# 21K1113/Neural_Image_Compression_V2

Measured on AMD Instinct MI355X. Metric: Mpixels/sec train-step (fwd+bwd) + PSNR, 4K RGB, 1/2/4/8 MI355X, higher is better.
Workload: dtype bf16x2-split operands, f32 accumulate

## Files before the change

### ab/w16/scratch_depth.py

```python
import re, sys, collections
kern, depth = None, 0
acc, mfma = collections.defaultdict(list), collections.defaultdict(collections.Counter)
for l in open(sys.argv[1]):
    m = re.match(r"^(_ZN3nic\w+):", l)
    if m:
        kern, depth = (re.sub(r".*LayoutILi(\d)EEELi(\d).*", r"Layout<\1>, MODE \2", m.group(1)) if "fused_train16" in m.group(1) else None), 0
        continue
    if kern is None:
        continue
    if re.match(r"^(\.LBB\d+_\d+:|; %bb\.\d+:)", l):
        d = re.search(r"Depth=(\d+)", l)
        depth = int(d.group(1)) if d else 0
    elif "scratch_" in l:
        acc[kern].append((depth, l.split()[0]))
    elif "v_mfma" in l:
        mfma[kern][depth] += 1
for k in mfma:
    print(f"{k}: MFMAs by depth {dict(mfma[k])}; scratch accesses by depth {dict(collections.Counter(d for d, _ in acc[k]))}"
          f"{'  <-- IN THE ROUND LOOP' if any(d >= 3 for d, _ in acc[k]) else ''}")
```

### ab/w16/stamps16.py

```python
import os, sys, ctypes
sys.path.insert(0, os.path.dirname(os.path.dirname(os.path.dirname(os.path.abspath(__file__)))))
import torch, numpy as np
from neural_image_compression_v2_amd import _lib, fused, fp_def
from neural_image_compression_v2_amd.image_compression import ColorDecoder
dev = torch.device("cuda:0")
torch.manual_seed(0)
H, W = 2160, 3840
NS = H * W
fp, _ = fp_def.create_pyramid((H // 4, W // 4), 12, 8, dev, torch.float32, True)
dec = ColorDecoder(73, 64).to(dev)
geo = fused.PathGeometry(dim=2, method=1, step_number=0.25, mip_level=0, extent=(H, W), num_crops=1,
                         noise_mode=int(os.environ.get("NOISE", "2")), noise_seed=7, noise_offset=1,
                         flags=_lib.NIC_FLAG_ORIGINS_ALIGNED, split_bf16=True)
org = torch.zeros(1, 2, dtype=torch.int32, device=dev)
params = [p.detach() for p in dec.linear_params()]
target = torch.rand(NS, 3, device=dev)
for _ in range(3):
    out = fused.fused_forward_backward(geo, fp[0].detach(), fp[1].detach(), org, params, target)
torch.cuda.synchronize()
d = geo.to_desc(fp[0], fp[1])
ws = _lib.workspace(dev, int(_lib.load().nic_workspace_bytes(ctypes.byref(d))))
REC, NWG = 20992, 256
off = NWG * REC * 4
st = ws[off:off + NWG * 8 * 16 * 8].view(torch.int64).view(NWG * 8, 16).cpu().numpy().astype(np.float64)
names = ["0 coords, blend, PE, noise", "1 L1, L2, L3 (+ image stores, GELUs)", "2 dZ3 image, dW3, dA2", "3 dA1 (+ dZ2 image), db2", "4 wait barrier 1",
         "5 dW2 MFMAs", "6 wait barrier 2", "7 dX (+ dZ1 image), grid acc", "8 wait barrier 3", "9 dW1 MFMAs", "10 wait barrier 4", "11 -",
         "12 macro-tile setup", "13 grid flush"]
tot = st[:, :14].sum(1)
print(f"waves {st.shape[0]}, total cycles/wave median {np.median(tot):.3e} (min {tot.min():.3e}, max {tot.max():.3e})")
rounds = NS / 16 / (NWG * 8)
for i, n in enumerate(names):
    print(f"{n:40s} {100 * np.median(st[:, i] / tot):6.2f} %   {np.median(st[:, i]) / rounds:9.0f} cycles/round")
wave_id = np.arange(st.shape[0]) % 8
for kh in (0, 1):
    sel = (wave_id >> 2) == kh
    print(f"-- half {kh}: total cycles/wave median {np.median(tot[sel]):.3e}")
    for i, n in enumerate(names):
        print(f"   {n:40s} {np.median(st[sel, i]) / rounds:9.0f} cycles/round")
```

### neural_image_compression_v2_amd/csrc/fused_train16.hpp

```cpp
#pragma once
#include "fused_kernel.hpp"


#ifndef NIC_T16_HALF16
#define NIC_T16_HALF16 1
#endif
#ifndef NIC_T16_LOFF
#define NIC_T16_LOFF 26
#endif
#ifndef NIC_T16_PIN
#define NIC_T16_PIN 0
#endif
namespace nic {

struct Lds16 {
    static constexpr int LD1 = 80, LD2 = 80, LD3 = 80;
    static constexpr int LDZ = 72, LDX = 88;
    static constexpr int KP = 80;
    static constexpr int OFF_W1 = 0;
    static constexpr int W1LO = kH * LD1;
    static constexpr int OFF_W2 = OFF_W1 + 2 * kH * LD1;
    static constexpr int W2LO = kH * LD2;
    static constexpr int OFF_W3 = OFF_W2 + 2 * kH * LD2;
    static constexpr int W3LO = 4 * LD3;
// ... 52 lines not shown
__device__ __forceinline__ Frag2 split_pair(const f32x4& a, const f32x4& b) {
    const float x[8] = {a[0], a[1], a[2], a[3], b[0], b[1], b[2], b[3]};
    return split8(x);
}
__device__ __forceinline__ lds_bf* opaque(lds_bf* p) {
#ifndef NIC_NO_OPAQUE_PTR
    asm volatile("" : "+v"(p));
#endif
    return p;
}

#ifndef NIC_T16_PF
#define NIC_T16_PF 2
#endif
template <int NT, bool ZERO = false, class LoadA>
__device__ __forceinline__ void kstep16(f32x4 (&acc)[NT], const Frag2& bf, LoadA&& load_a) {
    constexpr int PF = NIC_T16_PF < NT ? NIC_T16_PF : NT;
    Frag2 af[PF];
#pragma unroll
    for (int t = 0; t < PF; ++t) af[t] = load_a(t);
#pragma unroll
    for (int t = 0; t < NT; ++t) {
        acc[t] = mfma16_split(af[t % PF], bf, ZERO ? f32x4(0.f) : acc[t]);
        if (t + PF < NT) af[t % PF] = load_a(t + PF);
    }
}

struct CellRaw16 {
    float g0[kC];
    float g1[4 * 3];
};
struct GridAcc16 {
    float g1[4 * 3];
};

__device__ __forceinline__ int opaque_i(int v) {
#ifndef NIC_NO_OPAQUE_LANE
    asm volatile("" : "+v"(v));
#endif
    return v;
}

__device__ __forceinline__ float grid_load16(const char* base, uint32_t ob, int kind, const FusedParams& p) {
    if (kind == 0) return *reinterpret_cast<const float*>(base + ob);
    if (kind == 3) {
        const float n = (float)*reinterpret_cast<const uint8_t*>(base + ob) - p.dq_sub;
        const float q = mul_rn(n, p.dq_rcp);
        return fmaf(fmaf(-q, p.dq_den, n), p.dq_rcp, q);
    }
    const uint32_t hbits = *reinterpret_cast<const uint16_t*>(base + ob);
    if (kind == 1) return __builtin_bit_cast(float, hbits << 16);
    return (float)__builtin_bit_cast(_Float16, (uint16_t)hbits);
}
__device__ __forceinline__ void gather_cell16(const FusedParams& p, uint32_t off0, uint32_t off1, int g, CellRaw16& raw) {
    const int kind = p.grid_kind;
    const uint32_t eb = kind == 0 ? 4u : (kind == 3 ? 1u : 2u);
    const uint32_t pb0 = (uint32_t)p.g0.plane * eb, pb1 = (uint32_t)p.g1.plane * eb;
    {
        uint32_t ob = (off0 + (uint32_t)p.g0.at(g >> 1, g & 1, 0)) * eb;
        const char* base = reinterpret_cast<const char*>(p.g0.p);
#pragma unroll
        for (int c = 0; c < kC; ++c, ob += pb0) raw.g0[c] = grid_load16(base, ob, kind, p);
    }
#pragma unroll
    for (int c4 = 0; c4 < 4; ++c4) {
        uint32_t ob = (off1 + (uint32_t)p.g1.at(c4 >> 1, c4 & 1, 0)) * eb + (uint32_t)(3 * g) * pb1;
        const char* base = reinterpret_cast<const char*>(p.g1.p);
#pragma unroll
        for (int cc = 0; cc < 3; ++cc, ob += pb1) raw.g1[c4 * 3 + cc] = grid_load16(base, ob, kind, p);
    }
}

template <class L>
__device__ __forceinline__ void encode16(const FusedParams& p, const int (&q)[3], int g, float (&xs)[20], EncCtx& cx, const CellRaw16& raw) {
    const nic_path_desc& d = p.d;
    const int e = d.log2_step;
    const Axis ax = axis_coords(q[0], e), ay = axis_coords(q[1], e);
    cx.kx = ax.k1; cx.ky = ay.k1; cx.kz = 0.f;
#pragma unroll
    for (int c = 0; c < kC; ++c) xs[c] = raw.g0[c];
    {
        const float c = (g >> 1) ? ay.t1 : ax.t1;
#pragma unroll
        for (int i = 0; i < 3; ++i) {
            const int r = 3 * (g & 1) + i;
            float v;
            if (L::PE == NIC_PE_TRIANGULAR) {
                v = tri_pe_row(c, r, kP);
            } else {
                const int k = r >> 1;
                const float dv = k == 0 ? d.pe_div[0] : (k == 1 ? d.pe_div[1] : d.pe_div[2]);
                float sv, cv;
                sincos_cw(mul_rn(c, dv), sv, cv);
                v = (r & 1) ? cv : sv;
            }
            xs[15 + i] = v;
        }
        xs[18] = g == 0 ? d.lod_value : (g == 1 ? 1.0f : 0.f);
    }
    const G1FactorsT<2> gf = g1_factors<2>(d.g1_weight_mode, cx.kx, cx.ky, 0.f);
#pragma unroll
    for (int cc = 0; cc < 3; ++cc) {
        float sum = 0.f;
#pragma unroll
        for (int c4 = 0; c4 < 4; ++c4) {
            const uint32_t b = (gf.bits >> (3 * c4)) & 7u;
            float v = raw.g1[c4 * 3 + cc];
            v = mul_rn(v, (b & 1u) ? gf.fx[1] : gf.fx[0]);
            v = mul_rn(v, (b & 2u) ? gf.fy[1] : gf.fy[0]);
            sum = c4 == 0 ? v : add_rn(sum, v);
        }
        xs[12 + cc] = sum;
    }
}
__host__ __device__ constexpr int xs_of_slot(int s) { return s < 15 ? s : s - 1; }

template <class L>
__device__ __forceinline__ void add_noise16(const NoiseSrc& ns, uint64_t sample_global, int64_t n_local, int g, float (&xs)[20]) {
    if (ns.mode == NIC_NOISE_NONE) return;
    if (ns.mode == NIC_NOISE_TENSOR) {
        const float* row = ns.tensor + n_local * L::CIN;
#pragma unroll
        for (int s = 0; s < 20; ++s) {
            if (s == 15) continue;
            const int ch0 = slot16_channel(s, 0);
            if (s == 19) { xs[18] += g == 0 ? row[72] : 0.f; continue; }
            const int stride = slot16_channel(s, 1) - ch0;
            xs[xs_of_slot(s)] += row[ch0 + stride * g];
        }
        return;
    }
    const U4 b = noise_block(ns, sample_global, g);
#pragma unroll
    for (int f = 0; f < 18; ++f) xs[f] += noise_field(ns, b, f);
    const float nl = noise_field(ns, b, 18);
    xs[18] += g == 0 ? nl : 0.f;
}

__device__ __forceinline__ void combine_g1_lanes16(GridAcc16& ga, uint32_t off1, const int (&blk)[3], int lane, int lw) {
    const int T[2] = {1 << lw, 16 >> lw};
    const int STR[2] = {1, 1 << lw};
    const int pl = lane & 15;
    const int lc[2] = {pl & (T[0] - 1), pl >> lw};
#pragma unroll
    for (int a = 0; a < 2; ++a) {
        const bool odd = blk[a] & 1;
        const int pc = lc[a] + (odd ? -1 : 1);
        const bool inb = pc >= 0 && pc < T[a];
        const int partner = inb ? lane + (odd ? -STR[a] : STR[a]) : lane;
        const bool pair = inb && (uint32_t)__shfl((int)off1, partner) == off1;
#pragma unroll
        for (int i = 0; i < 12; ++i) {
            const float pv = __shfl(ga.g1[i], partner);
            ga.g1[i] = pair ? (odd ? 0.f : ga.g1[i] + pv) : ga.g1[i];
        }
    }
}

__device__ __forceinline__ void preadd_x16(f32x4 (&dxacc)[4], uint32_t off0, int ln) {
    const int n16 = ln & 15, g = ln >> 4;
    const bool recv = g < 2;
    const bool inb = recv ? n16 >= 1 : n16 <= 14;
    const int partner = inb ? (recv ? ln + 31 : ln - 31) : ln;
    const uint32_t poff = (uint32_t)__shfl((int)off0, partner);
    const bool pair = inb && (recv ? off0 == poff + 1u : poff == off0 + 1u);
#pragma unroll
    for (int c = 0; c < kC; ++c) {
        const float pv = __shfl(dxacc[c >> 2][c & 3], partner);
        dxacc[c >> 2][c & 3] = pair ? (recv ? dxacc[c >> 2][c & 3] + pv : 0.f) : dxacc[c >> 2][c & 3];
    }
}
template <int NW, class Barrier>
__device__ __forceinline__ void preadd_y16(f32x4 (&dxacc)[4], uint32_t off0, uint32_t row, int ln, int wave, lds_f* reg0, int region, Barrier&& barrier) {
    typedef __attribute__((address_space(3))) uint32_t lds_u32_t;
    const int g = ln >> 4;
    lds_f* const mine = opaque(reg0 + wave * region + ln);
    const bool up = (g & 1) != 0;
    ((lds_u32_t*)mine)[12 * 64] = off0;
    if (up) {
#pragma unroll
        for (int i = 0; i < 12; ++i) mine[i * 64] = dxacc[i >> 2][i & 3];
    }
    barrier();
    const int pw = up ? wave + 1 : wave - 1;
    const bool inw = pw >= 0 && pw < NW;
    lds_cf* const theirs = opaque(reg0 + (inw ? pw : wave) * region + (up ? ln - 16 : ln + 16));
    const uint32_t poff = ((const lds_u32_t*)theirs)[12 * 64];
    const bool pair = inw && (up ? poff == off0 + row : off0 == poff + row);
    if (!up) {
#pragma unroll
        for (int i = 0; i < 12; ++i) {
            const float pv = theirs[i * 64];
            dxacc[i >> 2][i & 3] += pair ? pv : 0.f;
        }
    } else {
#pragma unroll
        for (int i = 0; i < 12; ++i) dxacc[i >> 2][i & 3] = pair ? 0.f : dxacc[i >> 2][i & 3];
    }
    barrier();
}

#ifndef NIC_T16_PREADD
#define NIC_T16_PREADD 2
#endif
#ifndef NIC_T16_LB
#define NIC_T16_LB 512
#endif
constexpr int MODE_TRAIN_RGBX = 4;
template <class L, int MODE>
__global__ void __launch_bounds__(NIC_T16_LB) fused_train16_kernel(FusedParams p) {
    using S = Lds16;
    static_assert(L::DIM == 2 && L::CIN == 73, "the 16-sample training kernel is built for the 2D slot layouts");
    static_assert(MODE != MODE_INFER, "training kernel");
    constexpr int LD1 = S::LD1, LD2 = S::LD2, LD3 = S::LD3, LDZ = S::LDZ, LDX = S::LDX;
    __shared__ __attribute__((aligned(16))) __bf16 smem16[S::TOTAL];
    lds_bf* const sm = (lds_bf*)smem16;

    const int tid = threadIdx.x, lane = tid & 63;
    const int wave = __builtin_amdgcn_readfirstlane(tid >> 6);

    stage_all<kH * LD1, 512>(tid,
        [&](int idx) {
            const int o = idx / LD1, rho = idx - o * LD1;
            const int ch = channel_of_rho16(rho);
            const float* src = ch >= 0 ? &p.W[0][o * L::CIN + ch] : &p.b[0][o];
            const float v = *src;
            return (ch >= 0 || ch == kSlotOne) ? v : 0.f;
        },
        [&](int idx, float v) {
            const __bf16 hi = (__bf16)v;
            sm[S::OFF_W1 + idx] = hi;
            sm[S::OFF_W1 + S::W1LO + idx] = (__bf16)(v - (float)hi);
        });
    stage_all<kH * LD2, 512>(tid,
        [&](int idx) {
            const int o = idx / LD2, ps = idx - o * LD2;
            const float v = p.W[1][o * kH + hid16(ps < kH ? ps : 0)];
            return ps < kH ? v : 0.f;
        },
        [&](int idx, float v) {
            const __bf16 hi = (__bf16)v;
            sm[S::OFF_W2 + idx] = hi;
            sm[S::OFF_W2 + S::W2LO + idx] = (__bf16)(v - (float)hi);
        });
    stage_all<4 * LD3, 512>(tid,
        [&](int idx) {
            const int c = idx / LD3, ps = idx - c * LD3;
            return (c < 3 && ps < kH) ? p.W[2][c * kH + hid16(ps)] : 0.f;
        },
        [&](int idx, float v) {
            const __bf16 hi = (__bf16)v;
            sm[S::OFF_W3 + idx] = hi;
// ... 2 lines not shown
    lds_f* const Bs = (lds_f*)(sm + S::OFF_B);
    if (tid < kH) Bs[tid] = p.b[1][tid];
    if (tid >= kH && tid < kH + 4) Bs[tid] = tid - kH < 3 ? p.b[2][tid - kH] : 0.f;
    for (int idx = tid; idx < 8 * S::SPW / 2; idx += 512) ((lds_f*)(sm + S::OFF_IMG))[idx] = 0.f;
    __syncthreads();
    const NoiseSrc nsrc = noise_with_step(p.noise, p.step_dev);

    f32x16 accW2 = f32x16(0.f);
    f32x16 accW1 = f32x16(0.f);
    f32x4 accT = f32x4(0.f);
    f32x4 accW3q = f32x4(0.f), accB2q = f32x4(0.f);
    float accB3[3] = {0.f, 0.f, 0.f}, accLoss = 0.f;
    const int T4 = wave & 3, kh = wave >> 2;
    const int to = T4 >> 1, tk = T4 & 1;
    lds_bf* const img0 = sm + S::OFF_IMG;

#ifdef NIC_STAMPS
    unsigned long long stamp_sum[NIC_NPH];
#pragma unroll
    for (int i = 0; i < NIC_NPH; ++i) stamp_sum[i] = 0;
    unsigned long long stamp_last;
    asm volatile("s_memtime %0\n\ts_waitcnt lgkmcnt(0)" : "=s"(stamp_last)::"memory");
#endif

    constexpr int LOFF = NIC_T16_LOFF;
    int lo_rW = 0, lo_rZ = 0, lo_tW = 0, lo_b44 = 0, lo_tZ = 0, lo_rX = 0;
    {
        const int n16 = lane & 15, g = lane >> 4, q4 = (lane & 15) >> 2, p4 = lane & 3, h32 = lane >> 5, cg = (lane >> 4) & 1;
        if constexpr ((LOFF & 1) != 0) lo_rW = opaque_i(n16 * S::LD1 + 8 * g);
        if constexpr ((LOFF & 2) != 0) lo_rZ = opaque_i(wave * S::SPW + n16 * S::LDZ + 8 * g);
        if constexpr ((LOFF & 4) != 0) lo_tW = opaque_i((4 * g + q4) * S::LD1 + 8 * p4);
        if constexpr ((LOFF & 8) != 0) lo_b44 = opaque_i(wave * S::SPW + 4 * q4 * S::LDZ + 16 * g + 4 * p4);
        if constexpr ((LOFF & 16) != 0) lo_tZ = opaque_i((4 * (wave >> 2)) * S::SPW + (4 * q4 + 2 * h32) * S::LDZ + 16 * cg + 4 * p4);
        if constexpr ((LOFF & 32) != 0) lo_rX = opaque_i(wave * S::SPW + S::OFF_X + n16 * S::LDX + 8 * g);
    }
    const int xcd = blockIdx.x & 7, nb8 = gridDim.x >> 3;
  for (int seg = 0; seg < 2; ++seg) {
    const int seg_tile0 = seg ? (int)p.seg_split : 0;
    const int seg_tiles = seg ? (int)p.n_tiles - (int)p.seg_split : (int)p.seg_split;
    const int rg = seg ? p.rg_log2 : 0;
    if (seg_tiles <= 0) continue;
    const int n_units = seg_tiles << rg;
    const int chunk = (((n_units + 7) >> 3) + 7) & ~7;
    const int t_begin = xcd * chunk;
    const int t_end = t_begin + chunk < n_units ? t_begin + chunk : n_units;
    const int lstride = nb8 * 8;
    const int base0 = t_begin + (int)(blockIdx.x >> 3) * 8;
    const int n_my = base0 < t_end ? (t_end - base0 + lstride - 1) / lstride : 0;
    const int tiles_per_crop = (int)p.tiles_per_crop, tiles_main = (int)p.tiles_main;
    const int rounds_unit = (p.niter * p.passes) >> rg;
    const int nph = rounds_unit >= NIC_PHASES ? NIC_PHASES : (rounds_unit >= 2 ? 2 : 1);
    const int shift = (NIC_STAGGER && (NIC_STAGGER_RG || rg == 0)) ? (int)((blockIdx.x >> 3) & (nph - 1)) * (rounds_unit / nph) : 0;

    for (int kk = 0; kk < n_my + (shift ? 1 : 0); ++kk) {
        const int base = base0 + (kk < n_my ? kk : 0) * lstride;
        const bool tile_ok = base + wave < t_end;
        const int unit = tile_ok ? base + wave : t_end - 1;
        const int tile = seg_tile0 + (unit >> rg);
        int it_len = rounds_unit, it_begin = (int)(unit & ((1 << rg) - 1)) * rounds_unit;
        if (shift) {
            if (kk == 0) { it_begin += shift; it_len -= shift; }
            else if (kk == n_my) it_len = shift;
        }
        int lw = 4;
        int org[3] = {0, 0, 0}, blk[3] = {0, 0, 0};
        const int crop = tile / tiles_per_crop;
        GridAcc16 gacc;
        f32x4 dxacc[4];
        f32x4 sdz1[4];
        uint32_t blk_off0, blk_off1;
        CellRaw16 raw;
        {
            const int ln = opaque_i(lane), n16 = ln & 15, g = ln >> 4;
            const int tt = tile - crop * tiles_per_crop;
            int boff[2];
            if (p.edge_lw < 0 || tt < tiles_main) {
                boff[1] = tt % p.tiles_y;
                boff[0] = (tt / p.tiles_y) * 16;
            } else {
                lw = p.edge_lw;
                boff[1] = (tt - tiles_main) * (16 >> lw);
                boff[0] = p.full_x * 16;
            }
            const int lc[2] = {n16 & ((1 << lw) - 1), n16 >> lw};
#pragma unroll
            for (int a = 0; a < 2; ++a) {
                org[a] = origin_of(p, crop * 2 + a);
                blk[a] = (org[a] >> p.lm) + boff[a] + lc[a];
            }
#pragma unroll
            for (int i = 0; i < 12; ++i) gacc.g1[i] = 0.f;
#pragma unroll
            for (int t = 0; t < 4; ++t) { dxacc[t] = f32x4(0.f); sdz1[t] = f32x4(0.f); }
            const int qb[3] = {blk[0] << p.lm, blk[1] << p.lm, 0};
            cell_offsets<L>(p, qb, blk_off0, blk_off1);
            gather_cell16(p, blk_off0, blk_off1, g, raw);
        }
        STAMP(12);

        for (int it = it_begin; it < it_begin + it_len; ++it) {
            f32x4 a1[4], d1[4], a2[4], d2[4];
            float dz3[3];
            float kx1, ky1;
            {
                const int ln = opaque_i(lane), n16 = ln & 15, g = ln >> 4;
                bool valid = tile_ok;
                int64_t n;
                int q[3] = {0, 0, 0};
                {
                    const int m1 = (1 << p.lm) - 1;
                    const int pass = it >> (p.lm * 2), its = it & (p.niter - 1);
                    const int j[2] = {its >> p.lm, its & m1};
                    const int ext[2] = {p.d.extent[0], p.d.extent[1]};
                    int idx[2];
#pragma unroll
                    for (int a = 0; a < 2; ++a) {
                        const int i = (blk[a] << p.lm) + j[a] - org[a];
                        valid = valid && i >= 0 && i < ext[a];
                        idx[a] = i < 0 ? 0 : (i >= ext[a] ? ext[a] - 1 : i);
                        q[a] = org[a] + idx[a];
                    }
                    n = ((int64_t)crop * p.passes + pass) * p.n_per_crop + (int64_t)idx[0] * ext[1] + idx[1];
                }
                float tgt[3] = {0.f, 0.f, 0.f};
                if (MODE == MODE_TRAIN_RGBX) {
                    const uint32_t off = (uint32_t)q[0] * (uint32_t)p.timg_s[0] + (uint32_t)q[1] * (uint32_t)p.timg_s[1];
                    const uint32_t rgbx = reinterpret_cast<const uint32_t*>(p.timg)[off];
#pragma unroll
                    for (int c = 0; c < 3; ++c) {
                        const float u = (float)((rgbx >> (8 * c)) & 255u);
                        const float t0 = mul_rn(u, p.timg_rcp);
                        tgt[c] = fmaf(fmaf(-t0, p.timg_den, u), p.timg_rcp, t0);
                    }
                } else if (MODE == MODE_TRAIN_IMG) {
                    const int64_t off = (int64_t)q[0] * p.timg_s[0] + (int64_t)q[1] * p.timg_s[1];
                    uint32_t rgbx = 0u;
                    if (p.timg_u8 == 2) rgbx = reinterpret_cast<const uint32_t*>(p.timg)[off];
#pragma unroll
                    for (int c = 0; c < 3; ++c) {
                        if (p.timg_u8) {
                            const float u = p.timg_u8 == 2 ? (float)((rgbx >> (8 * c)) & 255u) : (float)(reinterpret_cast<const uint8_t*>(p.timg) + c * p.timg_cs)[off];
                            const float t0 = mul_rn(u, p.timg_rcp);
                            tgt[c] = fmaf(fmaf(-t0, p.timg_den, u), p.timg_rcp, t0);
                        } else {
                            tgt[c] = (reinterpret_cast<const float*>(p.timg) + c * p.timg_cs)[off];
                        }
                    }
                } else {
                    const float* tp = (MODE == MODE_TRAIN_MSE ? p.target : p.dy) + n * 3;
#pragma unroll
                    for (int c = 0; c < 3; ++c) tgt[c] = tp[c];
                }
                float xs[20];
                {
                    EncCtx cx;
                    encode16<L>(p, q, g, xs, cx, raw);
                    kx1 = cx.kx; ky1 = cx.ky;
                    add_noise16<L>(nsrc, (uint64_t)(p.d.sample_base + n), n, g, xs);
                }
                STAMP(0);
                lds_bf* const imgw = img0 + wave * S::SPW;
                {
                    lds_cbf* const w_row = opaque((lds_cbf*)(sm + ((LOFF & 1) ? lo_rW : n16 * LD1 + 8 * g)));
                    lds_cbf* const w1_row2 = opaque((lds_cbf*)(sm + S::OFF_W1 + 64 + ((LOFF & 1) ? lo_rW - 4 * g : n16 * LD1 + 4 * g)));
                    lds_bf* const x_st = (LOFF & 32) ? opaque(img0 + lo_rX) : opaque(imgw + S::OFF_X + n16 * LDX + 8 * g);
                    lds_bf* const x_st2 = (LOFF & 32) ? opaque(img0 + 64 + lo_rX - 4 * g) : opaque(imgw + S::OFF_X + n16 * LDX + 64 + 4 * g);
                    f32x4 z[4];
#pragma unroll
                    for (int s = 0; s < 2; ++s) {
                        const float xv[8] = {xs[8 * s], xs[8 * s + 1], xs[8 * s + 2], xs[8 * s + 3], xs[8 * s + 4], xs[8 * s + 5], xs[8 * s + 6],
                                             s == 0 ? xs[7] : 0.f};
                        const Frag2 bf = split8(xv);
                        st_frag(&x_st[32 * s], bf.hi);
                        st_frag(&x_st[S::XLO + 32 * s], bf.lo);
                        auto la = [&](int t) {
                            Frag2 a;
                            a.hi = ld_frag(&w_row[S::OFF_W1 + 16 * t * LD1 + 32 * s]);
                            a.lo = ld_frag(&w_row[S::OFF_W1 + S::W1LO + 16 * t * LD1 + 32 * s]);
                            return a;
                        };
                        if (s == 0) kstep16<4, true>(z, bf, la);
                        else kstep16<4>(z, bf, la);
                    }
                    {
                        const float xv[8] = {xs[15], xs[16], xs[17], xs[18], 0.f, 0.f, 0.f, 0.f};
                        const Frag2 bf = split8(xv);
                        const s16x8 bh = __builtin_bit_cast(s16x8, bf.hi), bl = __builtin_bit_cast(s16x8, bf.lo);
                        *reinterpret_cast<lds_s16x4*>(x_st2) = s16x4{bh[0], bh[1], bh[2], bh[3]};
                        *reinterpret_cast<lds_s16x4*>(x_st2 + S::XLO) = s16x4{bl[0], bl[1], bl[2], bl[3]};
#if NIC_T16_HALF16
                        const Half2 bq = {s16x4{bh[0], bh[1], bh[2], bh[3]}, s16x4{bl[0], bl[1], bl[2], bl[3]}};
#pragma unroll
                        for (int t = 0; t < 4; ++t) {
                            const Half2 a = {*reinterpret_cast<lds_cs16x4*>(&w1_row2[16 * t * LD1]), *reinterpret_cast<lds_cs16x4*>(&w1_row2[S::W1LO + 16 * t * LD1])};
                            z[t] = mfma16h_split(a, bq, z[t]);
                        }
#else
                        kstep16<4>(z, bf, [&](int t) {
                            Frag2 a;
                            a.hi = half_frag(*reinterpret_cast<lds_cs16x4*>(&w1_row2[16 * t * LD1]));
                            a.lo = half_frag(*reinterpret_cast<lds_cs16x4*>(&w1_row2[S::W1LO + 16 * t * LD1]));
                            return a;
                        });
#endif
                    }
#pragma unroll
                    for (int t = 0; t < 4; ++t) gelu_and_grad4(z[t], a1[t], d1[t]);
                    if (NIC_T16_PIN & 1) {
#pragma unroll
                        for (int t = 0; t < 4; ++t) asm volatile("" : "+v"(d1[t]));
                    }
                    lds_cf* const b2_row = opaque(Bs + 4 * g);
                    lds_bf* const a1_st = (LOFF & 2) ? opaque(img0 + S::OFF_A1 + lo_rZ) : opaque(imgw + S::OFF_A1 + n16 * LDZ + 8 * g);
#pragma unroll
                    for (int t = 0; t < 4; ++t) z[t] = ld4(&b2_row[16 * t]);
#pragma unroll
                    for (int s = 0; s < 2; ++s) {
                        const Frag2 bf = split_pair(a1[2 * s], a1[2 * s + 1]);
                        st_frag(&a1_st[32 * s], bf.hi);
                        st_frag(&a1_st[S::DZLO + 32 * s], bf.lo);
                        kstep16<4>(z, bf, [&](int t) {
                            Frag2 a;
                            a.hi = ld_frag(&w_row[S::OFF_W2 + 16 * t * LD2 + 32 * s]);
                            a.lo = ld_frag(&w_row[S::OFF_W2 + S::W2LO + 16 * t * LD2 + 32 * s]);
                            return a;
                        });
                    }
#pragma unroll
                    for (int t = 0; t < 4; ++t) gelu_and_grad4(z[t], a2[t], d2[t]);
                    if ((NIC_T16_PIN & 2) || ((NIC_T16_PIN & 4) && L::PE == NIC_PE_SINUSOIDAL)) {
#pragma unroll
                        for (int t = 0; t < 4; ++t) asm volatile("" : "+v"(d2[t]));
                    }
                }
                float yv[3];
                {
                    lds_cbf* const w3_row = opaque((lds_cbf*)(sm + S::OFF_W3 + (n16 < 3 ? n16 : 3) * LD3 + 8 * g));
                    lds_bf* const dz_st = (LOFF & 2) ? opaque(img0 + lo_rZ) : opaque(imgw + n16 * LDZ + 8 * g);
                    f32x4 z3;
#pragma unroll
                    for (int s = 0; s < 2; ++s) {
                        Frag2 af;
                        af.hi = ld_frag(&w3_row[32 * s]);
                        af.lo = ld_frag(&w3_row[S::W3LO + 32 * s]);
                        const Frag2 bf = split_pair(a2[2 * s], a2[2 * s + 1]);
                        st_frag(&dz_st[32 * s], bf.hi);
                        st_frag(&dz_st[S::DZLO + 32 * s], bf.lo);
                        z3 = mfma16_split(af, bf, s == 0 ? f32x4(0.f) : z3);
                    }
#pragma unroll
                    for (int c = 0; c < 3; ++c) yv[c] = sigmoid_f(z3[c] + ((lds_cf*)Bs)[kH + c]);
                }
                STAMP(1);
                const bool own = valid && g == 0;
                if (p.y != nullptr && own) {
#pragma unroll
                    for (int c = 0; c < 3; ++c) p.y[n * 3 + c] = yv[c];
                }
#pragma unroll
                for (int c = 0; c < 3; ++c) {
                    float gr;
                    if (MODE == MODE_TRAIN_MSE || MODE == MODE_TRAIN_IMG || MODE == MODE_TRAIN_RGBX) {
                        const float diff = own ? yv[c] - tgt[c] : 0.f;
                        accLoss += diff * diff;
                        gr = p.grad_scale * diff;
                    } else {
                        gr = own ? tgt[c] : 0.f;
                    }
                    dz3[c] = gr * yv[c] * (1.0f - yv[c]);
                    accB3[c] += dz3[c];
                }
                if (g == 0) {
                    lds_bf* const d3_st = opaque(imgw + S::OFF_D3 + 4 * (n16 & 3) + (n16 >> 2));
#pragma unroll
                    for (int c = 0; c < 3; ++c) {
                        const __bf16 hi = (__bf16)dz3[c];
                        d3_st[c * 16] = hi;
                        d3_st[64 + c * 16] = (__bf16)(dz3[c] - (float)hi);
                    }
                }
            }
            wave_lds_fence();
            f32x4 dz1[4];
            {
                const int ln = opaque_i(lane), n16 = ln & 15, g = ln >> 4, q4 = (ln & 15) >> 2, p4 = ln & 3;
                lds_bf* const imgw = img0 + wave * S::SPW;
                lds_cbf* const dz_b44 = (LOFF & 8) ? opaque((lds_cbf*)(img0 + lo_b44)) : opaque((lds_cbf*)(imgw + 4 * q4 * LDZ + 16 * g + 4 * p4));
                {
                    lds_cbf* const d3_a44 = opaque((lds_cbf*)(imgw + S::OFF_D3 + (ln & 3) * 16));
                    s16x4 bh[4], bl[4], ah[4], al[4];
#pragma unroll
                    for (int r = 0; r < 4; ++r) {
                        bh[r] = tr4(&dz_b44[r * LDZ]);
                        bl[r] = tr4(&dz_b44[S::DZLO + r * LDZ]);
                        ah[r] = *reinterpret_cast<lds_cs16x4*>(&d3_a44[4 * r]);
                        al[r] = *reinterpret_cast<lds_cs16x4*>(&d3_a44[64 + 4 * r]);
                    }
#pragma unroll
                    for (int r = 0; r < 4; ++r) {
                        accW3q = mfma4_bf(al[r], bh[r], accW3q);
                        accW3q = mfma4_bf(ah[r], bl[r], accW3q);
                        accW3q = mfma4_bf(ah[r], bh[r], accW3q);
                    }
                }
// ... 93 lines not shown
                    st_frag(&dz_st[32 * s], bf.hi);
                    st_frag(&dz_st[S::DZLO + 32 * s], bf.lo);
                    auto la = [&](int) {
                        constexpr int co = 32 * (3 >> 1) + 4 * (3 & 1);
                        Frag2 a;
                        a.hi = join8(tr4(&w1_tr[32 * s * LD1 + co]), tr4(&w1_tr[(32 * s + 16) * LD1 + co]));
                        a.lo = join8(tr4(&w1_tr[S::W1LO + 32 * s * LD1 + co]), tr4(&w1_tr[S::W1LO + (32 * s + 16) * LD1 + co]));
                        return a;
                    };
                    if (s == 0) kstep16<1, true>(dx3, bf, la);
                    else kstep16<1>(dx3, bf, la);
                }
                const G1FactorsT<2> gf = g1_factors<2>(p.d.g1_weight_mode, kx1, ky1, 0.f);
#pragma unroll
                for (int c4 = 0; c4 < 4; ++c4) {
                    const float w = g1_corner_factor<2>(gf, c4);
#pragma unroll
                    for (int cc = 0; cc < 3; ++cc) gacc.g1[c4 * 3 + cc] = fmaf(dx3[0][cc], w, gacc.g1[c4 * 3 + cc]);
                }
            }
            STAMP(7);
            wg_lds_barrier();
            STAMP(8);
            {
                const int ln = opaque_i(lane), g = ln >> 4, q4 = (ln & 15) >> 2, p4 = ln & 3, h32 = ln >> 5, cg = (ln >> 4) & 1;
                lds_cbf* const dz_t32 = opaque((lds_cbf*)(img0 + 32 * to + ((LOFF & 16) ? lo_tZ : (4 * kh) * S::SPW + (4 * q4 + 2 * h32) * LDZ + 16 * cg + 4 * p4)));
                lds_cbf* const x_t32 = opaque((lds_cbf*)(img0 + (4 * kh) * S::SPW + S::OFF_X + (4 * q4 + 2 * h32) * LDX + 32 * tk + 16 * cg + 4 * p4));
#pragma unroll
                for (int v = 0; v < 4; ++v) {
                    Frag2 af, bf;
                    af.hi = join8(tr4(&dz_t32[v * S::SPW]), tr4(&dz_t32[v * S::SPW + LDZ]));
                    bf.lo = join8(tr4(&x_t32[v * S::SPW + S::XLO]), tr4(&x_t32[v * S::SPW + S::XLO + LDX]));
                    af.lo = join8(tr4(&dz_t32[v * S::SPW + S::DZLO]), tr4(&dz_t32[v * S::SPW + S::DZLO + LDZ]));
                    bf.hi = join8(tr4(&x_t32[v * S::SPW]), tr4(&x_t32[v * S::SPW + LDX]));
                    accW1 = mfma_split(af, bf, accW1);
                }
                lds_cbf* const dz_t16 = opaque((lds_cbf*)(img0 + (4 * kh + (g >> 1)) * S::SPW + (4 * q4 + 2 * (g & 1)) * LDZ + 16 * T4 + 4 * p4));
                lds_cbf* const x_t16 = opaque((lds_cbf*)(img0 + (4 * kh + (g >> 1)) * S::SPW + S::OFF_X + (4 * q4 + 2 * (g & 1)) * LDX + 64 + 4 * p4));
#pragma unroll
                for (int uu = 0; uu < 2; ++uu) {
                    Frag2 af, bf;
                    af.hi = join8(tr4(&dz_t16[2 * uu * S::SPW]), tr4(&dz_t16[2 * uu * S::SPW + LDZ]));
                    af.lo = join8(tr4(&dz_t16[2 * uu * S::SPW + S::DZLO]), tr4(&dz_t16[2 * uu * S::SPW + S::DZLO + LDZ]));
                    bf.hi = join8(tr4(&x_t16[2 * uu * S::SPW]), tr4(&x_t16[2 * uu * S::SPW + LDX]));
                    bf.lo = join8(tr4(&x_t16[2 * uu * S::SPW + S::XLO]), tr4(&x_t16[2 * uu * S::SPW + S::XLO + LDX]));
                    accT = mfma16_split(af, bf, accT);
                }
            }
            STAMP(9);
            wg_lds_barrier();
            STAMP(10);
        }

        {
            const int ln = opaque_i(lane), g = ln >> 4, q4 = (ln & 15) >> 2, p4 = ln & 3;
            lds_cbf* const w1_tr = opaque((lds_cbf*)(sm + S::OFF_W1 + ((LOFF & 4) ? lo_tW : (4 * g + q4) * LD1 + 8 * p4)));
#pragma unroll
            for (int s = 0; s < 2; ++s) {
                const float x[8] = {sdz1[2 * s][0], sdz1[2 * s][1], sdz1[2 * s][2], sdz1[2 * s][3],
                                    sdz1[2 * s + 1][0], sdz1[2 * s + 1][1], sdz1[2 * s + 1][2], sdz1[2 * s + 1][3]};
                const Frag2 bf = split8(x);
                float r[8];
#pragma unroll
                for (int i = 0; i < 8; ++i) r[i] = (x[i] - (float)bf.hi[i]) - (float)bf.lo[i];
                const bf16x8 b3 = split8(r).hi;
#pragma unroll
                for (int t = 0; t < 3; ++t) {
                    const int co = 32 * (t >> 1) + 4 * (t & 1);
                    Frag2 a;
                    a.hi = join8(tr4(&w1_tr[32 * s * LD1 + co]), tr4(&w1_tr[(32 * s + 16) * LD1 + co]));
                    a.lo = join8(tr4(&w1_tr[S::W1LO + 32 * s * LD1 + co]), tr4(&w1_tr[S::W1LO + (32 * s + 16) * LD1 + co]));
                    f32x4 c = mfma16_bf(a.lo, bf.lo, s == 0 ? f32x4(0.f) : dxacc[t]);
                    c = mfma16_bf(a.hi, b3, c);
                    dxacc[t] = mfma16_split(a, bf, c);
                }
            }
        }
        {
            const int ln = opaque_i(lane), g = ln >> 4;
            combine_g1_lanes16(gacc, blk_off1, blk, ln, lw);
            bool flush = true;
            if (NIC_GROUP_SUM && rg > 0) {
                lds_f* const reg0 = (lds_f*)img0;
                constexpr int REGION = S::SPW / 2;
                static_assert(24 * 64 <= REGION, "group-sum scratch");
                int leader = wave;
                if (tile_ok)
                    for (int w = wave - 1; w >= 4 * kh; --w)
                        if (seg_tile0 + ((base + w) >> rg) == tile) leader = w;
                if (leader != wave) {
                    lds_f* const mine = opaque(reg0 + wave * REGION + ln);
#pragma unroll
                    for (int i = 0; i < 12; ++i) mine[i * 64] = dxacc[i >> 2][i & 3];
#pragma unroll
                    for (int i = 0; i < 12; ++i) mine[(12 + i) * 64] = gacc.g1[i];
                }
                wg_lds_barrier();
                if (leader == wave && tile_ok) {
                    for (int w = wave + 1; w < 4 * kh + 4; ++w) {
                        if (base + w >= t_end || seg_tile0 + ((base + w) >> rg) != tile) break;
                        lds_cf* const theirs = opaque(reg0 + w * REGION + ln);
#pragma unroll
                        for (int i = 0; i < 12; ++i) dxacc[i >> 2][i & 3] += theirs[i * 64];
#pragma unroll
                        for (int i = 0; i < 12; ++i) gacc.g1[i] += theirs[(12 + i) * 64];
                    }
                }
                wg_lds_barrier();
                flush = leader == wave;
            }
            if (flush && NIC_T16_PREADD) preadd_x16(dxacc, blk_off0, ln);
            if (NIC_T16_PREADD >= 2 && rg == 0 && (p.preadd_y || !NIC_PREADD_Y_SMALL)) {
                static_assert(13 * 64 <= S::SPW / 2, "pre-add scratch");
                preadd_y16<8>(dxacc, blk_off0, (uint32_t)p.g0.nx, ln, wave, (lds_f*)img0, S::SPW / 2, [&]() { wg_lds_barrier(); });
            }
            if (flush) {
                const uint32_t pb0 = (uint32_t)p.g0.plane * 4u, pb1 = (uint32_t)p.g1.plane * 4u;
                uint32_t nz0 = 0u, nz1 = 0u;
#pragma unroll
                for (int c = 0; c < kC; ++c) {
                    nz0 |= __builtin_bit_cast(uint32_t, dxacc[c >> 2][c & 3]);
                    nz1 |= __builtin_bit_cast(uint32_t, gacc.g1[c]);
                }
                if ((nz0 << 1) != 0u) {
                    uint32_t ob = (blk_off0 + (uint32_t)p.g0.at(g >> 1, g & 1, 0)) * 4u;
                    char* gbase = reinterpret_cast<char*>(p.g0_grad);
#pragma unroll
                    for (int c = 0; c < kC; ++c, ob += pb0) atomicAdd(reinterpret_cast<float*>(gbase + ob), dxacc[c >> 2][c & 3]);
                }
                if ((nz1 << 1) != 0u) {
#pragma unroll
                    for (int c4 = 0; c4 < 4; ++c4) {
                        uint32_t ob = (blk_off1 + (uint32_t)p.g1.at(c4 >> 1, c4 & 1, 0)) * 4u + (uint32_t)(3 * g) * pb1;
                        char* gbase = reinterpret_cast<char*>(p.g1_grad);
#pragma unroll
                        for (int cc = 0; cc < 3; ++cc, ob += pb1) atomicAdd(reinterpret_cast<float*>(gbase + ob), gacc.g1[c4 * 3 + cc]);
                    }
                }
            }
        }
        STAMP(13);
    }
  }
#ifdef NIC_STAMPS
    if (lane == 0) {
        unsigned long long* dst = reinterpret_cast<unsigned long long*>(p.partials + (size_t)gridDim.x * S::REC) + ((size_t)blockIdx.x * 8 + wave) * 16;
#pragma unroll
        for (int i = 0; i < NIC_NPH; ++i) dst[i] = stamp_sum[i];
    }
#endif

    float* rec = p.partials + (int64_t)blockIdx.x * S::REC;
#pragma unroll
    for (int r = 0; r < 16; ++r) {
        rec[S::REC_W2 + wave * 1024 + r * 64 + lane] = accW2[r];
        rec[S::REC_W1 + wave * 1024 + r * 64 + lane] = accW1[r];
    }
#pragma unroll
    for (int r = 0; r < 4; ++r) rec[S::REC_TAIL + wave * 256 + r * 64 + lane] = accT[r];
    float* tail = rec + S::REC_WAVE + wave * 320;
    tail[lane] = accB2q[0];
#pragma unroll
    for (int c = 0; c < 3; ++c) tail[64 + 64 * c + lane] = accW3q[c];
#pragma unroll
    for (int c = 0; c < 4; ++c) {
        float v = c < 3 ? accB3[c] : accLoss;
#pragma unroll
        for (int m = 32; m > 0; m >>= 1) v += __shfl_xor(v, m);
        if (lane == 0) tail[256 + c] = v;
    }
}

constexpr int kR16_SRC = 4096 + 4096 + 1024 + 320;
#ifndef NIC_R16_SLICES
#define NIC_R16_SLICES 8
#endif
template <class L>
__global__ void __launch_bounds__(256) reduce16_kernel(const float* partials, int n_rec, nic_mlp_grads gr, float* loss, float loss_scale, const StepTail tl) {
    if (tail_block(tl)) return;
    using S = Lds16;
    constexpr int SL = NIC_R16_SLICES, OUTS = 256 / SL;
    __shared__ float red[SL][OUTS];
    const int slice = threadIdx.x / OUTS, oi = threadIdx.x % OUTS;
    const int gid = blockIdx.x * OUTS + oi;
    const bool live = gid < kR16_SRC;
    int nsrc = 0, off0 = 0, stride = 0;
// ... 58 lines not shown
```

Before: 4010.

## Prefetch next unit's header and grid cell before the dW1 and flush phase

Moves the per-unit setup (tile coordinates, cell offsets, grid gather) into a helper and issues it for the next unit before the current unit's dW1 MFMAs and gradient flush, so the gather latency can overlap that work. A copy of the flushing unit's offsets is kept for the atomics. It also adds a grid_kind switch so each gather is specialised by element type, and replaces __shfl with ds_bpermute. The trade is higher register pressure, since the next unit's raw cell is live across the flush, which risks spills.

```diff
diff --git a/ab/w16/scratch_depth.py b/ab/w16/scratch_depth.py
--- a/ab/w16/scratch_depth.py
+++ b/ab/w16/scratch_depth.py
@@ -1,7 +1,8 @@
 import re, sys, collections
 kern, depth = None, 0
 acc, mfma = collections.defaultdict(list), collections.defaultdict(collections.Counter)
-for l in open(sys.argv[1]):
+lines = open(sys.argv[1]).read().split("\n")
+for i, l in enumerate(lines):
     m = re.match(r"^(_ZN3nic\w+):", l)
     if m:
         kern, depth = (re.sub(r".*LayoutILi(\d)EEELi(\d).*", r"Layout<\1>, MODE \2", m.group(1)) if "fused_train16" in m.group(1) else None), 0
@@ -9,12 +10,19 @@
     if kern is None:
         continue
     if re.match(r"^(\.LBB\d+_\d+:|; %bb\.\d+:)", l):
-        d = re.search(r"Depth=(\d+)", l)
+        head = [l]
+        for n in lines[i + 1:i + 12]:
+            if not n.lstrip().startswith(";"):
+                break
+            head.append(n)
+        own = [h for h in head if "Loop Header" in h] or [h for h in head if "in Loop:" in h]
+        d = re.search(r"Depth=(\d+)", own[0]) if own else None
         depth = int(d.group(1)) if d else 0
     elif "scratch_" in l:
         acc[kern].append((depth, l.split()[0]))
     elif "v_mfma" in l:
         mfma[kern][depth] += 1
 for k in mfma:
+    rd = max(mfma[k], key=lambda d: mfma[k][d])
     print(f"{k}: MFMAs by depth {dict(mfma[k])}; scratch accesses by depth {dict(collections.Counter(d for d, _ in acc[k]))}"
-          f"{'  <-- IN THE ROUND LOOP' if any(d >= 3 for d, _ in acc[k]) else ''}")
+          f"{'  <-- IN THE ROUND LOOP' if any(d >= rd for d, _ in acc[k]) else ''}")
diff --git a/ab/w16/stamps16.py b/ab/w16/stamps16.py
--- a/ab/w16/stamps16.py
+++ b/ab/w16/stamps16.py
@@ -24,13 +24,27 @@
 off = NWG * REC * 4
 st = ws[off:off + NWG * 8 * 16 * 8].view(torch.int64).view(NWG * 8, 16).cpu().numpy().astype(np.float64)
 names = ["0 coords, blend, PE, noise", "1 L1, L2, L3 (+ image stores, GELUs)", "2 dZ3 image, dW3, dA2", "3 dA1 (+ dZ2 image), db2", "4 wait barrier 1",
-         "5 dW2 MFMAs", "6 wait barrier 2", "7 dX (+ dZ1 image), grid acc", "8 wait barrier 3", "9 dW1 MFMAs", "10 wait barrier 4", "11 -",
+         "5 dW2 MFMAs", "6 wait barrier 2", "7 dX (+ dZ1 image), grid acc", "8 wait barrier 3", "9 dW1 MFMAs", "10 wait barrier 4", "11 phase 0 of a unit's first round",
          "12 macro-tile setup", "13 grid flush"]
 tot = st[:, :14].sum(1)
 print(f"waves {st.shape[0]}, total cycles/wave median {np.median(tot):.3e} (min {tot.min():.3e}, max {tot.max():.3e})")
 rounds = NS / 16 / (NWG * 8)
 for i, n in enumerate(names):
     print(f"{n:40s} {100 * np.median(st[:, i] / tot):6.2f} %   {np.median(st[:, i]) / rounds:9.0f} cycles/round")
+RU = 16
+units = rounds / RU
+ph0_first, ph0_rest = np.median(st[:, 11]) / units, np.median(st[:, 0]) / (rounds - units)
+summary = {"cycles_per_wave": float(np.median(tot)), "units_per_wave": units,
+           "per_round": {n: float(np.median(st[:, i]) / rounds) for i, n in enumerate(names)},
+           "setup_per_unit": float(np.median(st[:, 12]) / units), "flush_per_unit": float(np.median(st[:, 13]) / units),
+           "phase0_first_round": float(ph0_first), "phase0_other_rounds": float(ph0_rest), "first_round_surplus_per_unit": float(ph0_first - ph0_rest)}
+summary["boundary_share"] = (summary["setup_per_unit"] + summary["flush_per_unit"] + summary["first_round_surplus_per_unit"]) * units / summary["cycles_per_wave"]
+print(f"per unit: setup {summary['setup_per_unit']:.0f}, flush {summary['flush_per_unit']:.0f}, phase 0 first round {ph0_first:.0f} / other rounds {ph0_rest:.0f} cycles; "
+      f"boundary + first-round surplus = {100 * summary['boundary_share']:.2f} % of a wave's cycles")
+if os.environ.get("STAMPS_JSON"):
+    import json
+    with open(os.environ["STAMPS_JSON"], "w") as f:
+        json.dump(summary, f, indent=1)
 wave_id = np.arange(st.shape[0]) % 8
 for kh in (0, 1):
     sel = (wave_id >> 2) == kh
diff --git a/neural_image_compression_v2_amd/csrc/fused_train16.hpp b/neural_image_compression_v2_amd/csrc/fused_train16.hpp
--- a/neural_image_compression_v2_amd/csrc/fused_train16.hpp
+++ b/neural_image_compression_v2_amd/csrc/fused_train16.hpp
@@ -128,8 +128,7 @@
     if (kind == 1) return __builtin_bit_cast(float, hbits << 16);
     return (float)__builtin_bit_cast(_Float16, (uint16_t)hbits);
 }
-__device__ __forceinline__ void gather_cell16(const FusedParams& p, uint32_t off0, uint32_t off1, int g, CellRaw16& raw) {
-    const int kind = p.grid_kind;
+__device__ __forceinline__ void gather_cell16_kind(const FusedParams& p, const int kind, uint32_t off0, uint32_t off1, int g, CellRaw16& raw) {
     const uint32_t eb = kind == 0 ? 4u : (kind == 3 ? 1u : 2u);
     const uint32_t pb0 = (uint32_t)p.g0.plane * eb, pb1 = (uint32_t)p.g1.plane * eb;
     {
@@ -144,6 +143,17 @@
         const char* base = reinterpret_cast<const char*>(p.g1.p);
 #pragma unroll
         for (int cc = 0; cc < 3; ++cc, ob += pb1) raw.g1[c4 * 3 + cc] = grid_load16(base, ob, kind, p);
+    }
+}
+__device__ __forceinline__ void gather_cell16(const FusedParams& p, uint32_t off0, uint32_t off1, int g, CellRaw16& raw) {
+    gather_cell16_kind(p, p.grid_kind, off0, off1, g, raw);
+}
+__device__ __forceinline__ void gather_cell16_switched(const FusedParams& p, uint32_t off0, uint32_t off1, int g, CellRaw16& raw) {
+    switch (p.grid_kind) {
+        case 0: gather_cell16_kind(p, 0, off0, off1, g, raw); break;
+        case 1: gather_cell16_kind(p, 1, off0, off1, g, raw); break;
+        case 3: gather_cell16_kind(p, 3, off0, off1, g, raw); break;
+        default: gather_cell16_kind(p, 2, off0, off1, g, raw); break;
     }
 }
 
@@ -213,6 +223,8 @@
     xs[18] += g == 0 ? nl : 0.f;
 }
 
+__device__ __forceinline__ int shfl_lane(int v, int src_lane) { return __builtin_amdgcn_ds_bpermute(src_lane << 2, v); }
+__device__ __forceinline__ float shfl_lane(float v, int src_lane) { return __builtin_bit_cast(float, __builtin_amdgcn_ds_bpermute(src_lane << 2, __builtin_bit_cast(int, v))); }
 __device__ __forceinline__ void combine_g1_lanes16(GridAcc16& ga, uint32_t off1, const int (&blk)[3], int lane, int lw) {
     const int T[2] = {1 << lw, 16 >> lw};
     const int STR[2] = {1, 1 << lw};
@@ -224,10 +236,10 @@
         const int pc = lc[a] + (odd ? -1 : 1);
         const bool inb = pc >= 0 && pc < T[a];
         const int partner = inb ? lane + (odd ? -STR[a] : STR[a]) : lane;
-        const bool pair = inb && (uint32_t)__shfl((int)off1, partner) == off1;
+        const bool pair = inb && (uint32_t)shfl_lane((int)off1, partner) == off1;
 #pragma unroll
         for (int i = 0; i < 12; ++i) {
-            const float pv = __shfl(ga.g1[i], partner);
+            const float pv = shfl_lane(ga.g1[i], partner);
             ga.g1[i] = pair ? (odd ? 0.f : ga.g1[i] + pv) : ga.g1[i];
         }
     }
@@ -238,11 +250,11 @@
     const bool recv = g < 2;
     const bool inb = recv ? n16 >= 1 : n16 <= 14;
     const int partner = inb ? (recv ? ln + 31 : ln - 31) : ln;
-    const uint32_t poff = (uint32_t)__shfl((int)off0, partner);
+    const uint32_t poff = (uint32_t)shfl_lane((int)off0, partner);
     const bool pair = inb && (recv ? off0 == poff + 1u : poff == off0 + 1u);
 #pragma unroll
     for (int c = 0; c < kC; ++c) {
-        const float pv = __shfl(dxacc[c >> 2][c & 3], partner);
+        const float pv = shfl_lane(dxacc[c >> 2][c & 3], partner);
         dxacc[c >> 2][c & 3] = pair ? (recv ? dxacc[c >> 2][c & 3] + pv : 0.f) : dxacc[c >> 2][c & 3];
     }
 }
@@ -274,6 +286,62 @@
         for (int i = 0; i < 12; ++i) dxacc[i >> 2][i & 3] = pair ? 0.f : dxacc[i >> 2][i & 3];
     }
     barrier();
+}
+
+struct Seg16 {
+    int tile0, rg, t_end, base0, lstride, n_my, tiles_per_crop, tiles_main, rounds_unit, shift;
+};
+struct Unit16 {
+    int org[3], blk[3];
+    int qb[2];
+    int lw, crop;
+    int base, tile;
+    int it_begin, it_len;
+    bool tile_ok;
+    uint32_t blk_off0, blk_off1;
+    CellRaw16 raw;
+};
+struct UnitFlush16 {
+    int blk[3], lw, base, tile;
+    bool tile_ok;
+    uint32_t blk_off0, blk_off1;
+};
+template <class L>
+__device__ __forceinline__ void unit_header16(const FusedParams& p, const Seg16& sg, int kk, int lane, int wave, Unit16& u) {
+    u.base = sg.base0 + (kk < sg.n_my ? kk : 0) * sg.lstride;
+    u.tile_ok = u.base + wave < sg.t_end;
+    const int unit = u.tile_ok ? u.base + wave : sg.t_end - 1;
+    u.tile = sg.tile0 + (unit >> sg.rg);
+    u.it_len = sg.rounds_unit;
+    u.it_begin = (int)(unit & ((1 << sg.rg) - 1)) * sg.rounds_unit;
+    if (sg.shift) {
+        if (kk == 0) { u.it_begin += sg.shift; u.it_len -= sg.shift; }
+        else if (kk == sg.n_my) u.it_len = sg.shift;
+    }
+    u.lw = 4;
+    u.crop = u.tile / sg.tiles_per_crop;
+    const int ln = opaque_i(lane), n16 = ln & 15, g = ln >> 4;
+    const int tt = u.tile - u.crop * sg.tiles_per_crop;
+    int boff[2];
+    if (p.edge_lw < 0 || tt < sg.tiles_main) {
+        boff[1] = tt % p.tiles_y;
+        boff[0] = (tt / p.tiles_y) * 16;
+    } else {
+        u.lw = p.edge_lw;
+        boff[1] = (tt - sg.tiles_main) * (16 >> u.lw);
+        boff[0] = p.full_x * 16;
+    }
+    const int lc[2] = {n16 & ((1 << u.lw) - 1), n16 >> u.lw};
+#pragma unroll
+    for (int a = 0; a < 2; ++a) {
+        u.org[a] = origin_of(p, u.crop * 2 + a);
+        u.blk[a] = (u.org[a] >> p.lm) + boff[a] + lc[a];
+    }
+    u.org[2] = 0; u.blk[2] = 0;
+    u.qb[0] = u.blk[0] << p.lm; u.qb[1] = u.blk[1] << p.lm;
+    const int qb[3] = {u.qb[0], u.qb[1], 0};
+    cell_offsets<L>(p, qb, u.blk_off0, u.blk_off1);
+    gather_cell16_switched(p, u.blk_off0, u.blk_off1, g, u.raw);
 }
 
 #ifndef NIC_T16_PREADD
@@ -382,59 +450,30 @@
     const int nph = rounds_unit >= NIC_PHASES ? NIC_PHASES : (rounds_unit >= 2 ? 2 : 1);
     const int shift = (NIC_STAGGER && (NIC_STAGGER_RG || rg == 0)) ? (int)((blockIdx.x >> 3) & (nph - 1)) * (rounds_unit / nph) : 0;
 
-    for (int kk = 0; kk < n_my + (shift ? 1 : 0); ++kk) {
-        const int base = base0 + (kk < n_my ? kk : 0) * lstride;
-        const bool tile_ok = base + wave < t_end;
-        const int unit = tile_ok ? base + wave : t_end - 1;
-        const int tile = seg_tile0 + (unit >> rg);
-        int it_len = rounds_unit, it_begin = (int)(unit & ((1 << rg) - 1)) * rounds_unit;
-        if (shift) {
-            if (kk == 0) { it_begin += shift; it_len -= shift; }
-            else if (kk == n_my) it_len = shift;
-        }
-        int lw = 4;
-        int org[3] = {0, 0, 0}, blk[3] = {0, 0, 0};
-        const int crop = tile / tiles_per_crop;
+    const Seg16 sg = {seg_tile0, rg, t_end, base0, lstride, n_my, tiles_per_crop, tiles_main, rounds_unit, shift};
+    const int n_pieces = n_my + (shift ? 1 : 0);
+    Unit16 u;
+    if (n_pieces > 0) unit_header16<L>(p, sg, 0, lane, wave, u);
+    STAMP(12);
+
+    for (int kk = 0; kk < n_pieces; ++kk) {
         GridAcc16 gacc;
         f32x4 dxacc[4];
         f32x4 sdz1[4];
-        uint32_t blk_off0, blk_off1;
-        CellRaw16 raw;
-        {
-            const int ln = opaque_i(lane), n16 = ln & 15, g = ln >> 4;
-            const int tt = tile - crop * tiles_per_crop;
-            int boff[2];
-            if (p.edge_lw < 0 || tt < tiles_main) {
-                boff[1] = tt % p.tiles_y;
-                boff[0] = (tt / p.tiles_y) * 16;
-            } else {
-                lw = p.edge_lw;
-                boff[1] = (tt - tiles_main) * (16 >> lw);
-                boff[0] = p.full_x * 16;
-            }
-            const int lc[2] = {n16 & ((1 << lw) - 1), n16 >> lw};
-#pragma unroll
-            for (int a = 0; a < 2; ++a) {
-                org[a] = origin_of(p, crop * 2 + a);
-                blk[a] = (org[a] >> p.lm) + boff[a] + lc[a];
-            }
-#pragma unroll
-            for (int i = 0; i < 12; ++i) gacc.g1[i] = 0.f;
-#pragma unroll
-            for (int t = 0; t < 4; ++t) { dxacc[t] = f32x4(0.f); sdz1[t] = f32x4(0.f); }
-            const int qb[3] = {blk[0] << p.lm, blk[1] << p.lm, 0};
-            cell_offsets<L>(p, qb, blk_off0, blk_off1);
-            gather_cell16(p, blk_off0, blk_off1, g, raw);
-        }
-        STAMP(12);
-
-        for (int it = it_begin; it < it_begin + it_len; ++it) {
+        float zero = 0.f;
+        asm volatile("" : "+v"(zero));
+#pragma unroll
+        for (int i = 0; i < 12; ++i) gacc.g1[i] = zero;
+#pragma unroll
+        for (int t = 0; t < 4; ++t) { dxacc[t] = f32x4(zero); sdz1[t] = f32x4(zero); }
+
+        for (int it = u.it_begin; it < u.it_begin + u.it_len; ++it) {
             f32x4 a1[4], d1[4], a2[4], d2[4];
             float dz3[3];
             float kx1, ky1;
             {
                 const int ln = opaque_i(lane), n16 = ln & 15, g = ln >> 4;
-                bool valid = tile_ok;
+                bool valid = u.tile_ok;
                 int64_t n;
                 int q[3] = {0, 0, 0};
                 {
@@ -445,12 +484,12 @@
                     int idx[2];
 #pragma unroll
                     for (int a = 0; a < 2; ++a) {
-                        const int i = (blk[a] << p.lm) + j[a] - org[a];
+                        const int i = u.qb[a] + j[a] - u.org[a];
                         valid = valid && i >= 0 && i < ext[a];
                         idx[a] = i < 0 ? 0 : (i >= ext[a] ? ext[a] - 1 : i);
-                        q[a] = org[a] + idx[a];
-                    }
-                    n = ((int64_t)crop * p.passes + pass) * p.n_per_crop + (int64_t)idx[0] * ext[1] + idx[1];
+                        q[a] = u.org[a] + idx[a];
+                    }
+                    n = ((int64_t)u.crop * p.passes + pass) * p.n_per_crop + (int64_t)idx[0] * ext[1] + idx[1];
                 }
                 float tgt[3] = {0.f, 0.f, 0.f};
                 if (MODE == MODE_TRAIN_RGBX) {
@@ -484,11 +523,12 @@
                 float xs[20];
                 {
                     EncCtx cx;
-                    encode16<L>(p, q, g, xs, cx, raw);
+                    encode16<L>(p, q, g, xs, cx, u.raw);
                     kx1 = cx.kx; ky1 = cx.ky;
                     add_noise16<L>(nsrc, (uint64_t)(p.d.sample_base + n), n, g, xs);
                 }
-                STAMP(0);
+                if (it == u.it_begin) STAMP(11);
+                else STAMP(0);
                 lds_bf* const imgw = img0 + wave * S::SPW;
                 {
                     lds_cbf* const w_row = opaque((lds_cbf*)(sm + ((LOFF & 1) ? lo_rW : n16 * LD1 + 8 * g)));
@@ -578,8 +618,9 @@
                         st_frag(&dz_st[S::DZLO + 32 * s], bf.lo);
                         z3 = mfma16_split(af, bf, s == 0 ? f32x4(0.f) : z3);
                     }
-#pragma unroll
-                    for (int c = 0; c < 3; ++c) yv[c] = sigmoid_f(z3[c] + ((lds_cf*)Bs)[kH + c]);
+                    lds_cf* const b3_row = opaque(Bs + kH);
+#pragma unroll
+                    for (int c = 0; c < 3; ++c) yv[c] = sigmoid_f(z3[c] + b3_row[c]);
                 }
                 STAMP(1);
                 const bool own = valid && g == 0;
@@ -779,6 +820,11 @@
             STAMP(10);
         }
 
+        UnitFlush16 fu = {{u.blk[0], u.blk[1], 0}, u.lw, u.base, u.tile, u.tile_ok, u.blk_off0, u.blk_off1};
+        asm volatile("" : "+v"(fu.blk_off0), "+v"(fu.blk_off1), "+v"(fu.blk[0]), "+v"(fu.blk[1]));
+        if (kk + 1 < n_pieces) unit_header16<L>(p, sg, kk + 1, lane, wave, u);
+        STAMP(12);
+
         {
             const int ln = opaque_i(lane), g = ln >> 4, q4 = (ln & 15) >> 2, p4 = ln & 3;
             lds_cbf* const w1_tr = opaque((lds_cbf*)(sm + S::OFF_W1 + ((LOFF & 4) ? lo_tW : (4 * g + q4) * LD1 + 8 * p4)));
@@ -805,16 +851,16 @@
         }
         {
             const int ln = opaque_i(lane), g = ln >> 4;
-            combine_g1_lanes16(gacc, blk_off1, blk, ln, lw);
+            combine_g1_lanes16(gacc, fu.blk_off1, fu.blk, ln, fu.lw);
             bool flush = true;
             if (NIC_GROUP_SUM && rg > 0) {
                 lds_f* const reg0 = (lds_f*)img0;
                 constexpr int REGION = S::SPW / 2;
                 static_assert(24 * 64 <= REGION, "group-sum scratch");
                 int leader = wave;
-                if (tile_ok)
+                if (fu.tile_ok)
                     for (int w = wave - 1; w >= 4 * kh; --w)
-                        if (seg_tile0 + ((base + w) >> rg) == tile) leader = w;
+                        if (seg_tile0 + ((fu.base + w) >> rg) == fu.tile) leader = w;
                 if (leader != wave) {
                     lds_f* const mine = opaque(reg0 + wave * REGION + ln);
 #pragma unroll
@@ -823,9 +869,9 @@
                     for (int i = 0; i < 12; ++i) mine[(12 + i) * 64] = gacc.g1[i];
                 }
                 wg_lds_barrier();
-                if (leader == wave && tile_ok) {
+                if (leader == wave && fu.tile_ok) {
                     for (int w = wave + 1; w < 4 * kh + 4; ++w) {
-                        if (base + w >= t_end || seg_tile0 + ((base + w) >> rg) != tile) break;
+                        if (fu.base + w >= t_end || seg_tile0 + ((fu.base + w) >> rg) != fu.tile) break;
                         lds_cf* const theirs = opaque(reg0 + w * REGION + ln);
 #pragma unroll
                         for (int i = 0; i < 12; ++i) dxacc[i >> 2][i & 3] += theirs[i * 64];
@@ -836,10 +882,10 @@
                 wg_lds_barrier();
                 flush = leader == wave;
             }
-            if (flush && NIC_T16_PREADD) preadd_x16(dxacc, blk_off0, ln);
+            if (flush && NIC_T16_PREADD) preadd_x16(dxacc, fu.blk_off0, ln);
             if (NIC_T16_PREADD >= 2 && rg == 0 && (p.preadd_y || !NIC_PREADD_Y_SMALL)) {
                 static_assert(13 * 64 <= S::SPW / 2, "pre-add scratch");
-                preadd_y16<8>(dxacc, blk_off0, (uint32_t)p.g0.nx, ln, wave, (lds_f*)img0, S::SPW / 2, [&]() { wg_lds_barrier(); });
+                preadd_y16<8>(dxacc, fu.blk_off0, (uint32_t)p.g0.nx, ln, wave, (lds_f*)img0, S::SPW / 2, [&]() { wg_lds_barrier(); });
             }
             if (flush) {
                 const uint32_t pb0 = (uint32_t)p.g0.plane * 4u, pb1 = (uint32_t)p.g1.plane * 4u;
@@ -850,7 +896,7 @@
                     nz1 |= __builtin_bit_cast(uint32_t, gacc.g1[c]);
                 }
                 if ((nz0 << 1) != 0u) {
-                    uint32_t ob = (blk_off0 + (uint32_t)p.g0.at(g >> 1, g & 1, 0)) * 4u;
+                    uint32_t ob = (fu.blk_off0 + (uint32_t)p.g0.at(g >> 1, g & 1, 0)) * 4u;
                     char* gbase = reinterpret_cast<char*>(p.g0_grad);
 #pragma unroll
                     for (int c = 0; c < kC; ++c, ob += pb0) atomicAdd(reinterpret_cast<float*>(gbase + ob), dxacc[c >> 2][c & 3]);
@@ -858,7 +904,7 @@
                 if ((nz1 << 1) != 0u) {
 #pragma unroll
                     for (int c4 = 0; c4 < 4; ++c4) {
-                        uint32_t ob = (blk_off1 + (uint32_t)p.g1.at(c4 >> 1, c4 & 1, 0)) * 4u + (uint32_t)(3 * g) * pb1;
+                        uint32_t ob = (fu.blk_off1 + (uint32_t)p.g1.at(c4 >> 1, c4 & 1, 0)) * 4u + (uint32_t)(3 * g) * pb1;
                         char* gbase = reinterpret_cast<char*>(p.g1_grad);
 #pragma unroll
                         for (int cc = 0; cc < 3; ++cc, ob += pb1) atomicAdd(reinterpret_cast<float*>(gbase + ob), gacc.g1[c4 * 3 + cc]);
```

After: 4129, median of 6. 3.0% higher.
